# JuliaSmoothOptimizers/LinearOperators.jl

Hardware: AMD Instinct MI355X
Metric: mul! GB/s (frac HBM peak) at n=10^8 fp64; L-BFGS apply/s, 1/2/4/8 GPU (higher is better)
Workload: dtype f64; 1 GPU; opHouseholder(h) 5-arg mul!(res,H,v,1,0), n=100000000 fp64 per GPU (configs[1]); n_per_gpu=100000000, algorithmic_bytes_per_elt=40, devices_visible=1

## Files before the change

linearoperators.jl_amd/csrc/house_keep.h:

```cpp
#pragma once
#include "common.h"
#include "house_keep_plan.h"
#include "stream_kernels.h"

namespace mxlo {

constexpr int kHouseKeepKR = 14;
constexpr int kHouseKeepKL = 4;
constexpr int kHouseKeepUnroll = 4;
static_assert(kHouseKeepUnroll == kStreamUnroll, "the dot launch and the update launch count the same chunks");

constexpr int kHouseResidentNum = 14;
static_assert(kHouseResidentNum >= 0 && kHouseResidentNum <= 16);
#define MXLO_POLICY_SIDE(tag) asm volatile("; h loads: " tag ::: "memory")
struct HouseResident {
  int q = 0;
  int grid = 0;
};

template <typename T, typename CA, typename CB, bool BETA0, int KR, int KL>
__global__ void __launch_bounds__(kBlock)
householder_dots_keep_kernel(T *__restrict__ res, const T *__restrict__ h, const T *__restrict__ v, int64_t head,
                             int64_t n, CA alpha, CB beta, HouseKeepPlan pl, unsigned long long *__restrict__ slots,
                             unsigned long long ticks, unsigned *__restrict__ fault, int drop,
                             double *__restrict__ dot_out, int rq) {
  constexpr int VEC = Vec16<T>::N, U = kHouseKeepUnroll;
  using V = typename Vec16<T>::type;
  constexpr int64_t CHUNK = (int64_t)kBlock * U;
  extern __shared__ __attribute__((aligned(16))) unsigned char keep_lds[];
  V *lh = reinterpret_cast<V *>(keep_lds), *lx = lh + (int64_t)KL * CHUNK;
  const int tid = threadIdx.x, G = (int)gridDim.x, b = (int)blockIdx.x;
  GridExchange X;
  X.begin<kBlock>(slots, kFusedSlots);

  const V *hv = reinterpret_cast<const V *>(h + head), *xv = reinterpret_cast<const V *>(v + head);
  V *rv = reinterpret_cast<V *>(res + head);
  double acc = 0.0;
  auto load4 = [&](int64_t round, V (&a)[U], V (&x)[U]) {
    const int64_t base = (round * G + b) * CHUNK + tid;
    if (house_resident_diag((int)((round + b) & 15), rq)) {
      MXLO_POLICY_SIDE("resident");
#pragma unroll
      for (int u = 0; u < U; ++u) {
        x[u] = __builtin_nontemporal_load(xv + base + (int64_t)u * kBlock);
        a[u] = hv[base + (int64_t)u * kBlock];
      }
      MXLO_POLICY_SIDE("resident, issued");
    } else {
      MXLO_POLICY_SIDE("streamed");
#pragma unroll
      for (int u = 0; u < U; ++u) {
        x[u] = __builtin_nontemporal_load(xv + base + (int64_t)u * kBlock);
        a[u] = __builtin_nontemporal_load(hv + base + (int64_t)u * kBlock);
      }
      MXLO_POLICY_SIDE("streamed, issued");
    }
  };
  auto fma4 = [&](const V (&a)[U], const V (&x)[U]) {
#pragma unroll
    for (int u = 0; u < U; ++u)
#pragma unroll
      for (int k = 0; k < VEC; ++k) acc = fma((double)a[u][k], (double)x[u][k], acc);
  };
  for (int64_t r = 0; r < pl.first; ++r) {
    V a[U], x[U];
    load4(r, a, x);
    fma4(a, x);
  }
  if constexpr (KL > 0) {
#pragma unroll 1
    for (int q = 0; q < pl.kl; ++q) {
      V a[U], x[U];
      load4(pl.first + q, a, x);
      fma4(a, x);
#pragma unroll
      for (int u = 0; u < U; ++u) {
        lh[(q * U + u) * kBlock + tid] = a[u];
        lx[(q * U + u) * kBlock + tid] = x[u];
      }
    }
  }
  V kh[KR][U], kx[KR][U];
  const int64_t reg0 = pl.first + pl.kl;
#pragma unroll
  for (int q = 0; q < KR; ++q)
    if (q < pl.kr) load4(reg0 + q, kh[q], kx[q]);
#pragma unroll
  for (int q = 0; q < KR; ++q)
    if (q < pl.kr) fma4(kh[q], kx[q]);
  const int64_t rem = pl.rem_vec + (int64_t)b * CHUNK + tid;
#pragma unroll
  for (int u = 0; u < U; ++u) {
    const int64_t i = rem + (int64_t)u * kBlock;
    if (i < pl.nvec) {
      const V x = __builtin_nontemporal_load(xv + i), a = __builtin_nontemporal_load(hv + i);
#pragma unroll
      for (int k = 0; k < VEC; ++k) acc = fma((double)a[k], (double)x[k], acc);
    }
  }
  const int64_t tail0 = head + pl.nvec * VEC, cnt = head + (n - tail0);
  if (b == G - 1 && tid < cnt) {
    const int64_t i = tid < head ? tid : tail0 + (tid - head);
    acc = fma((double)h[i], (double)v[i], acc);
  }

  __shared__ double lds[kBlock / kWave];
  const double s = block_sum4(acc, lds);
  if (tid == 0) X.publish(b, s, b == drop);
  double p = 0.0;
  for (int i = tid; i < G; i += kBlock) p += X.wait(i, ticks, fault, kFaultHouseholder);
  __syncthreads();
  const double dot = block_sum4(p, lds);
  if (b == 0 && tid == 0) *dot_out = dot;
  X.finish();

  HouseholderOp<T, CA, CB, BETA0> op{alpha, beta, nullptr, T(0)};
  op.c = (T)2 * (T)dot;
  auto update4 = [&](int64_t round, const V (&a)[U], const V (&x)[U]) {
    const int64_t base = (round * G + b) * CHUNK + tid;
    V r[U];
    if constexpr (!BETA0) {
#pragma unroll
      for (int u = 0; u < U; ++u) r[u] = __builtin_nontemporal_load(rv + base + (int64_t)u * kBlock);
    }
#pragma unroll
    for (int u = 0; u < U; ++u) {
      V o;
#pragma unroll
      for (int k = 0; k < VEC; ++k) o[k] = op(a[u][k], x[u][k], BETA0 ? T(0) : r[u][k]);
      __builtin_nontemporal_store(o, rv + base + (int64_t)u * kBlock);
    }
  };
#pragma unroll
  for (int q = 0; q < KR; ++q)
    if (q < pl.kr) update4(reg0 + q, kh[q], kx[q]);
  if constexpr (KL > 0) {
#pragma unroll 1
    for (int q = 0; q < pl.kl; ++q) {
      V a[U], x[U];
#pragma unroll
      for (int u = 0; u < U; ++u) {
        a[u] = lh[(q * U + u) * kBlock + tid];
        x[u] = lx[(q * U + u) * kBlock + tid];
      }
      update4(pl.first + q, a, x);
    }
  }
#pragma unroll
  for (int u = 0; u < U; ++u) {
    const int64_t i = rem + (int64_t)u * kBlock;
    if (i < pl.nvec) {
      const V x = xv[i], a = hv[i];
      V r, o;
      if constexpr (!BETA0) r = rv[i];
#pragma unroll
      for (int k = 0; k < VEC; ++k) o[k] = op(a[k], x[k], BETA0 ? T(0) : r[k]);
      __builtin_nontemporal_store(o, rv + i);
    }
  }
  if (b == G - 1 && tid >= head && tid < cnt) {
    const int64_t i = tail0 + (tid - head);
    res[i] = op(h[i], v[i], BETA0 ? T(0) : res[i]);
  }
}

template <typename T>
static int32_t householder_dots_t(mxlo_ctx *ctx, T *res, const T *h, const T *v, int64_t *n_left, double alpha,
                                  double beta, int32_t flags, double *dot, HouseResident *rs) {
  constexpr int VEC = Vec16<T>::N, KR = kHouseKeepKR, KL = kHouseKeepKL;
  constexpr int64_t CHUNK = (int64_t)kBlock * kHouseKeepUnroll;
  constexpr size_t kLds = (size_t)2 * KL * CHUNK * 16;
  const int64_t n = *n_left;
  const T *cols[1] = {h};
  const int64_t head = common_head<T>({res, h, v});
  bool keep = ctx->tune.house_fused && !ctx->allreduce && ctx->fault_dev && n > ctx->tune.house_inline_n && head >= 0 &&
              n >= 4 * VEC && (int64_t)sizeof(T) * n * 2 >= ctx->tune.nt_min_bytes;
  HouseKeepPlan pl;
  int grid = 0;
  if (keep) {
    const int per_cu = ctx->tune.red_blocks_per_cu > 1 ? 1 : ctx->tune.red_blocks_per_cu;
    grid = grid_for(ctx, (n - head) / VEC, CHUNK, per_cu);
    pl = house_keep_plan(n, head, VEC, grid, CHUNK, KR, KL);
    keep = grid == ctx->num_cu && grid <= kFusedSlots && pl.ok;
  }
  if (!keep) return panel_dots<T>(ctx, cols, 1, v, n, dot);
  const int rq = house_resident_q((int64_t)sizeof(T) * n, ctx->tune.nt_min_bytes / 16 * kHouseResidentNum);
  bool launched = false;
  MXLO_TRY((dispatch_ab<T>(beta, flags, [&]<typename CA, typename CB, bool B0>() -> int32_t {
    constexpr auto kernel = householder_dots_keep_kernel<T, CA, CB, B0, KR, KL>;
    static std::atomic<int> lds_cap[64];
    const int d = ctx->device & 63;
    int st = kLds > 48 * 1024 ? lds_cap[d].load(std::memory_order_relaxed) : 1;
    if (st == 0) {
      st = hipFuncSetAttribute((const void *)kernel, hipFuncAttributeMaxDynamicSharedMemorySize, (int)kLds) == hipSuccess ? 1 : 2;
      if (st == 2) (void)hipGetLastError();
      lds_cap[d].store(st, std::memory_order_relaxed);
    }
    if (st != 1 || !coresident<kernel>(ctx, grid, kLds)) return MXLO_OK;
    hipLaunchKernelGGL(kernel, dim3(grid), dim3(kBlock), kLds, ctx->stream, res, h, v, head, n, (CA)alpha, (CB)beta, pl,
                       ctx->xslots, fused_timeout_ticks(ctx), ctx->fault_dev, ctx->tune.fused_debug_drop, dot, rq);
    MXLO_LAUNCH_CHECK();
    launched = true;
    return MXLO_OK;
  })));
  if (!launched) return panel_dots<T>(ctx, cols, 1, v, n, dot);
  *n_left = pl.prefix;
  *rs = HouseResident{rq, grid};
  return MXLO_OK;
}

template <typename T, typename CA, typename CB, bool BETA0, bool REVERSE, bool NT>
__global__ void __launch_bounds__(kBlock)
householder_update_resident_kernel(T *__restrict__ res, const T *__restrict__ h, const T *__restrict__ v, int64_t head,
                                   int64_t nchunks, int64_t dots_grid, int rq, HouseholderOp<T, CA, CB, BETA0> op) {
  constexpr int VEC = Vec16<T>::N, U = kStreamUnroll;
  using V = typename Vec16<T>::type;
  constexpr int64_t CHUNK = (int64_t)kBlock * U;
  op.init();
  const int tid = threadIdx.x;
  V *rv = reinterpret_cast<V *>(res + head);
  const V *hv = reinterpret_cast<const V *>(h + head), *xv = reinterpret_cast<const V *>(v + head);
  for (int64_t ch = blockIdx.x; ch < nchunks; ch += gridDim.x) {
    const int64_t c = REVERSE ? (nchunks - 1 - ch) : ch;
    const int64_t base = c * CHUNK + tid;
    V a[U], x[U], r[U];
    if (house_resident_chunk(c, dots_grid, rq)) {
      MXLO_POLICY_SIDE("resident");
#pragma unroll
      for (int u = 0; u < U; ++u) {
        a[u] = hv[base + (int64_t)u * kBlock];
        x[u] = ldg<NT>(xv + base + (int64_t)u * kBlock);
        if constexpr (!BETA0) r[u] = ldg<NT>(rv + base + (int64_t)u * kBlock);
      }
      MXLO_POLICY_SIDE("resident, issued");
    } else {
      MXLO_POLICY_SIDE("streamed");
#pragma unroll
      for (int u = 0; u < U; ++u) {
        a[u] = ldg<NT>(hv + base + (int64_t)u * kBlock);
        x[u] = ldg<NT>(xv + base + (int64_t)u * kBlock);
        if constexpr (!BETA0) r[u] = ldg<NT>(rv + base + (int64_t)u * kBlock);
      }
      MXLO_POLICY_SIDE("streamed, issued");
    }
#pragma unroll
    for (int u = 0; u < U; ++u) {
      V o;
#pragma unroll
      for (int k = 0; k < VEC; ++k) o[k] = op(a[u][k], x[u][k], BETA0 ? T(0) : r[u][k]);
      stg<NT>(rv + base + (int64_t)u * kBlock, o);
    }
  }
  if (blockIdx.x == gridDim.x - 1 && tid < head) res[tid] = op(h[tid], v[tid], BETA0 ? T(0) : res[tid]);
}

template <typename T>
static int32_t householder_apply_resident_t(mxlo_ctx *ctx, T *res, const T *h, const T *v, int64_t n, double alpha,
                                            double beta, int32_t flags, const double *dot, HouseResident rs) {
  constexpr int VEC = Vec16<T>::N;
  constexpr int64_t CHUNK = (int64_t)kBlock * kStreamUnroll;
  const int64_t head = common_head<T>({res, h, v}), nchunks = (n - head) / VEC / CHUNK;
  MXLO_REQUIRE(head >= 0 && rs.grid > 0 && head + nchunks * CHUNK * VEC == n, MXLO_ESTATE,
               "householder: the prefix of the kept form is not the scalar head and whole chunks");
  const bool rev = ctx->tune.house_reverse != 0;
  int64_t g = nchunks;
  if (ctx->tune.blocks_per_cu > 0 && g > (int64_t)ctx->num_cu * ctx->tune.blocks_per_cu) g = (int64_t)ctx->num_cu * ctx->tune.blocks_per_cu;
  const int grid = (int)(g > 0x7fffffffLL ? 0x7fffffffLL : (g < 1 ? 1 : g));
  return dispatch_ab<T>(beta, flags, [&]<typename CA, typename CB, bool B0>() -> int32_t {
    HouseholderOp<T, CA, CB, B0> op{(CA)alpha, (CB)beta, dot, T(0)};
    const bool nt = (int64_t)sizeof(T) * n * (B0 ? 3 : 4) >= ctx->tune.nt_min_bytes;
    auto go = [&]<bool REV, bool NT>() {
      hipLaunchKernelGGL((householder_update_resident_kernel<T, CA, CB, B0, REV, NT>), dim3(grid), dim3(kBlock), 0,
                         ctx->stream, res, h, v, head, nchunks, (int64_t)rs.grid, rs.q, op);
    };
    if (rev) nt ? go.template operator()<true, true>() : go.template operator()<true, false>();
    else nt ? go.template operator()<false, true>() : go.template operator()<false, false>();
    MXLO_LAUNCH_CHECK();
    return MXLO_OK;
  });
}

}
```

linearoperators.jl_amd/csrc/house_keep_plan.h:

```cpp
#pragma once
#include <cstdint>

namespace mxlo {

struct HouseKeepPlan {
  bool ok = false;
  int64_t rounds = 0;
  int64_t first = 0;
  int kl = 0, kr = 0;
  int64_t prefix = 0;
  int64_t rem_vec = 0;
  int64_t nvec = 0;
};

inline HouseKeepPlan house_keep_plan(int64_t n, int64_t head, int vec, int64_t grid, int64_t chunk, int KR, int KL) {
  HouseKeepPlan p;
  if (n < head || vec < 1 || grid < 1 || chunk < 1 || KR < 0 || KL < 0) return p;
  p.nvec = (n - head) / vec;
  p.rounds = p.nvec / chunk / grid;
  if (p.rounds < 2) return p;
  const int64_t kept = p.rounds - 1 < (int64_t)KR + KL ? p.rounds - 1 : (int64_t)KR + KL;
  p.kr = (int)(kept < KR ? kept : KR);
  p.kl = (int)(kept - p.kr);
  p.first = p.rounds - kept;
  p.prefix = head + p.first * grid * chunk * vec;
  p.rem_vec = p.rounds * grid * chunk;
  p.ok = kept >= 1;
  return p;
}


constexpr int house_resident_q(int64_t h_bytes, int64_t cache_bytes) {
  if (cache_bytes <= 0 || h_bytes < 0) return 0;
  if (h_bytes <= cache_bytes) return 16;
  return (int)(cache_bytes / ((h_bytes + 15) / 16));
}

constexpr bool house_resident_diag(int t, int q) { return (t * q) % 16 >= 16 - q; }
constexpr bool house_resident_chunk(int64_t c, int64_t grid, int q) {
  return house_resident_diag((int)(((c / grid) + (c % grid)) % 16), q);
}

}
```

linearoperators.jl_amd/csrc/leaves.hip:

```cpp
#include "common.h"
#include "stream_kernels.h"
#include "house_keep.h"
using namespace mxlo;

#define CHECK_COMMON(name)                                                                       \
  MXLO_REQUIRE(ctx != nullptr, MXLO_EINVAL, name ": ctx is NULL");                               \
  MXLO_REQUIRE(dtype == MXLO_F64 || dtype == MXLO_F32, MXLO_EINVAL, name ": bad dtype %d", dtype)

static inline double eff_beta(int32_t dtype, int32_t flags, double beta) {
  return beta_is_f64(dtype == MXLO_F64 ? 8 : 4, flags) ? beta : (double)(float)beta;
}
static inline double eff_alpha(int32_t dtype, int32_t flags, double alpha) {
  return alpha_is_f64(dtype == MXLO_F64 ? 8 : 4, flags) ? alpha : (double)(float)alpha;
}

template <typename T>
static int32_t fill(mxlo_ctx *ctx, T *p, int64_t n, T c) {
  if (n <= 0) return MXLO_OK;
  if (c == T(0)) {
    MXLO_HIP(hipMemsetAsync(p, 0, sizeof(T) * (size_t)n, ctx->stream));
    return MXLO_OK;
  }
  return launch_map<T, 0, false, false>(ctx, p, (const T *)nullptr, (const T *)nullptr, n,
                                        FillOp<T>{c});
// ... 25 lines not shown
               "mxlo_diag_mul: NULL operand");
  const int64_t es = dtype == MXLO_F64 ? 8 : 4;
  MXLO_TRY(stage_alias(ctx, res, nrow * es, &v, n_min * es, true, "mxlo_diag_mul"));
  alpha = eff_alpha(dtype, flags, alpha);
  beta = eff_beta(dtype, flags, beta);
  if (dtype == MXLO_F64)
    return diag_mul_t<double>(ctx, (double *)res, (const double *)d, (const double *)v, n_min, nrow,
                              alpha, beta, flags);
  return diag_mul_t<float>(ctx, (float *)res, (const float *)d, (const float *)v, n_min, nrow,
                           alpha, beta, flags);
}

template <typename T>
static int32_t eye_mul_t(mxlo_ctx *ctx, T *res, const T *v, int64_t n_min, int64_t nrow,
                         double alpha, double beta, int32_t flags) {
  int32_t st = dispatch_ab<T>(beta, flags, [&]<typename CA, typename CB, bool B0>() -> int32_t {
    AxpbyOp<T, CA, CB, B0> op{(CA)alpha, (CB)beta};
    return launch_map<T, 1, !B0, false>(ctx, res, v, (const T *)nullptr, n_min, op);
  });
  MXLO_TRY(st);
  const int64_t ntail = nrow - n_min;
  if (ntail <= 0) return MXLO_OK;
  if (beta == 0) return fill<T>(ctx, res + n_min, ntail, T(0));
  const bool f64s = beta_is_f64(sizeof(T), flags);
  if (flags & MXLO_TAIL_BETA) return fill<T>(ctx, res + n_min, ntail, (T)beta);
  if (f64s)
    return launch_map<T, 0, true, false>(ctx, res + n_min, (const T *)nullptr, (const T *)nullptr,
                                         ntail, ScaleOp<T, double>{beta});
  return launch_map<T, 0, true, false>(ctx, res + n_min, (const T *)nullptr, (const T *)nullptr,
                                       ntail, ScaleOp<T, float>{(float)beta});
}

MXLO_API int32_t mxlo_eye_mul(mxlo_ctx *ctx, int32_t dtype, void *res, const void *v,
                              int64_t n_min, int64_t nrow, double alpha, double beta,
                              int32_t flags) {
  CHECK_COMMON("mxlo_eye_mul");
  MXLO_DEVICE_GUARD(ctx);
  MXLO_REQUIRE(n_min >= 0 && nrow >= n_min, MXLO_ESHAPE, "mxlo_eye_mul: n_min=%lld nrow=%lld",
               (long long)n_min, (long long)nrow);
  MXLO_REQUIRE(nrow == 0 || (res && (n_min == 0 || v)), MXLO_EINVAL, "mxlo_eye_mul: NULL operand");
  const int64_t es = dtype == MXLO_F64 ? 8 : 4;
  MXLO_TRY(stage_alias(ctx, res, nrow * es, &v, n_min * es, true, "mxlo_eye_mul"));
  alpha = eff_alpha(dtype, flags, alpha);
  beta = eff_beta(dtype, flags, beta);
  if (dtype == MXLO_F64)
    return eye_mul_t<double>(ctx, (double *)res, (const double *)v, n_min, nrow, alpha, beta, flags);
  return eye_mul_t<float>(ctx, (float *)res, (const float *)v, n_min, nrow, alpha, beta, flags);
}

template <typename T>
static int32_t scale_t(mxlo_ctx *ctx, T *res, int64_t n, double s, bool f64s) {
  if (f64s)
    return launch_map<T, 0, true, false>(ctx, res, (const T *)nullptr, (const T *)nullptr, n,
                                         ScaleOp<T, double>{s});
  return launch_map<T, 0, true, false>(ctx, res, (const T *)nullptr, (const T *)nullptr, n,
                                       ScaleOp<T, float>{(float)s});
}

MXLO_API int32_t mxlo_zeros_mul(mxlo_ctx *ctx, int32_t dtype, void *res, int64_t nrow, double beta,
                                int32_t flags) {
  CHECK_COMMON("mxlo_zeros_mul");
  MXLO_DEVICE_GUARD(ctx);
  MXLO_REQUIRE(nrow >= 0 && (nrow == 0 || res), MXLO_EINVAL, "mxlo_zeros_mul: bad argument");
  beta = eff_beta(dtype, flags, beta);
  if (beta == 0) {
    if (dtype == MXLO_F64) return fill<double>(ctx, (double *)res, nrow, 0.0);
    return fill<float>(ctx, (float *)res, nrow, 0.f);
  }
  if (dtype == MXLO_F64) return scale_t<double>(ctx, (double *)res, nrow, beta, true);
  return scale_t<float>(ctx, (float *)res, nrow, beta, beta_is_f64(4, flags));
}

MXLO_API int32_t mxlo_fill(mxlo_ctx *ctx, int32_t dtype, void *res, int64_t n, double value) {
  CHECK_COMMON("mxlo_fill");
  MXLO_DEVICE_GUARD(ctx);
  MXLO_REQUIRE(n >= 0 && (n == 0 || res), MXLO_EINVAL, "mxlo_fill: bad argument");
  if (dtype == MXLO_F64) return fill<double>(ctx, (double *)res, n, value);
  return fill<float>(ctx, (float *)res, n, (float)value);
}

MXLO_API int32_t mxlo_scale(mxlo_ctx *ctx, int32_t dtype, void *res, int64_t n, double alpha,
                            int32_t flags) {
  CHECK_COMMON("mxlo_scale");
  MXLO_DEVICE_GUARD(ctx);
  MXLO_REQUIRE(n >= 0 && (n == 0 || res), MXLO_EINVAL, "mxlo_scale: bad argument");
  alpha = eff_alpha(dtype, flags, alpha);
  if (dtype == MXLO_F64) return scale_t<double>(ctx, (double *)res, n, alpha, true);
  return scale_t<float>(ctx, (float *)res, n, alpha, alpha_is_f64(4, flags));
}

namespace {
template <typename T>
__global__ void __launch_bounds__(kBlock)
sum_kernel(const T *__restrict__ v, int64_t n, double *__restrict__ partials) {
  constexpr int VEC = Vec16<T>::N;
  using V = typename Vec16<T>::type;
  double acc = 0.0;
  const int64_t head = (((uintptr_t)v & 15u) == 0) ? 0 : n;
  const int64_t nvec = head == 0 ? n / VEC : 0;
  const V *vv = reinterpret_cast<const V *>(v);
  const int64_t stride = (int64_t)gridDim.x * kBlock;
  int64_t i = (int64_t)blockIdx.x * kBlock + threadIdx.x;
  for (; i + 3 * stride < nvec; i += 4 * stride) {
    const V a = __builtin_nontemporal_load(vv + i), b = __builtin_nontemporal_load(vv + i + stride),
            c = __builtin_nontemporal_load(vv + i + 2 * stride), d = __builtin_nontemporal_load(vv + i + 3 * stride);
#pragma unroll
    for (int e = 0; e < VEC; ++e) acc += ((double)a[e] + (double)b[e]) + ((double)c[e] + (double)d[e]);
  }
  for (; i < nvec; i += stride) {
    const V a = vv[i];
#pragma unroll
    for (int e = 0; e < VEC; ++e) acc += (double)a[e];
  }
  for (int64_t k = nvec * VEC + (int64_t)blockIdx.x * kBlock + threadIdx.x; k < n; k += stride) acc += (double)v[k];
#pragma unroll
  for (int off = 32; off > 0; off >>= 1) acc += __shfl_down(acc, off, 64);
  __shared__ double lds[kBlock / kWave];
  if ((threadIdx.x & 63) == 0) lds[threadIdx.x >> 6] = acc;
  __syncthreads();
  if (threadIdx.x == 0) partials[blockIdx.x] = (lds[0] + lds[1]) + (lds[2] + lds[3]);
}
}

namespace mxlo {
int32_t allreduce_hook(mxlo_ctx *ctx, double *dev, int64_t count);
}

template <typename T>
static int32_t ones_mul_t(mxlo_ctx *ctx, T *res, int64_t nrow, const T *v, int64_t ncol,
                          double alpha, double beta, int32_t flags) {
  double *sum = ctx->scalars;
  if (ncol > 0) {
    const int grid = grid_for(ctx, ncol, kBlock * 8, ctx->tune.red_blocks_per_cu);
    hipLaunchKernelGGL((sum_kernel<T>), dim3(grid), dim3(kBlock), 0, ctx->stream, v, ncol,
                       ctx->partials);
    MXLO_LAUNCH_CHECK();
    MXLO_TRY(finalize_and_reduce(ctx, 1, grid, sum));
  } else {
    MXLO_HIP(hipMemsetAsync(sum, 0, sizeof(double), ctx->stream));
  }
  MXLO_TRY(allreduce_hook(ctx, sum, 1));
  return dispatch_ab<T>(beta, flags, [&]<typename CA, typename CB, bool B0>() -> int32_t {
    OnesOp<T, CA, CB, B0> op{(CA)alpha, (CB)beta, sum, (CA)0};
    return launch_map<T, 0, !B0, false>(ctx, res, (const T *)nullptr, (const T *)nullptr, nrow, op);
  });
}

MXLO_API int32_t mxlo_ones_mul(mxlo_ctx *ctx, int32_t dtype, void *res, int64_t nrow,
                               const void *v, int64_t ncol, double alpha, double beta,
                               int32_t flags) {
  CHECK_COMMON("mxlo_ones_mul");
  MXLO_DEVICE_GUARD(ctx);
  MXLO_REQUIRE(nrow >= 0 && ncol >= 0, MXLO_ESHAPE, "mxlo_ones_mul: negative size");
  alpha = eff_alpha(dtype, flags, alpha);
  beta = eff_beta(dtype, flags, beta);
  if (dtype == MXLO_F64)
    return ones_mul_t<double>(ctx, (double *)res, nrow, (const double *)v, ncol, alpha, beta, flags);
  return ones_mul_t<float>(ctx, (float *)res, nrow, (const float *)v, ncol, alpha, beta, flags);
}

template <typename T>
static int32_t householder_apply_t(mxlo_ctx *ctx, T *res, const T *h, const T *v, int64_t n,
                                   double alpha, double beta, int32_t flags, const double *dot) {
  const bool rev = ctx->tune.house_reverse != 0;
  return dispatch_ab<T>(beta, flags, [&]<typename CA, typename CB, bool B0>() -> int32_t {
    HouseholderOp<T, CA, CB, B0> op{(CA)alpha, (CB)beta, dot, T(0)};
    if (rev) return launch_map<T, 2, !B0, true>(ctx, res, h, v, n, op);
    return launch_map<T, 2, !B0, false>(ctx, res, h, v, n, op);
  });
}

namespace {
template <typename T, typename CA, typename CB, bool BETA0, int VPT, bool ALIGNED>
__global__ void __launch_bounds__(kBlock)
householder_fused_kernel(T *__restrict__ res, const T *__restrict__ h, const T *__restrict__ v, int64_t n, CA alpha,
                         CB beta, unsigned long long *__restrict__ slots, unsigned long long ticks,
                         unsigned *__restrict__ fault, int drop) {
  constexpr int VEC = Vec16<T>::N;
  using V = typename Vec16<T>::type;
  const int tid = threadIdx.x, G = (int)gridDim.x, b = (int)blockIdx.x;
  GridExchange X;
  X.begin<kBlock>(slots, kFusedSlots);

  T hh[VPT][VEC], vv[VPT][VEC];
  double acc = 0.0;
  const int64_t base = (int64_t)b * kBlock * VPT * VEC;
#pragma unroll
  for (int q = 0; q < VPT; ++q) {
    const int64_t i = base + ((int64_t)q * kBlock + tid) * VEC;
    if (ALIGNED && i + VEC <= n) {
      const V a = *reinterpret_cast<const V *>(h + i), c = *reinterpret_cast<const V *>(v + i);
#pragma unroll
      for (int k = 0; k < VEC; ++k) { hh[q][k] = a[k]; vv[q][k] = c[k]; }
    } else {
#pragma unroll
      for (int k = 0; k < VEC; ++k) {
        hh[q][k] = i + k < n ? h[i + k] : T(0);
        vv[q][k] = i + k < n ? v[i + k] : T(0);
      }
    }
  }
#pragma unroll
  for (int q = 0; q < VPT; ++q)
#pragma unroll
    for (int k = 0; k < VEC; ++k) acc = fma((double)hh[q][k], (double)vv[q][k], acc);

  __shared__ double lds[kBlock / kWave];
  const double s = block_sum4(acc, lds);
  if (tid == 0) X.publish(b, s, b == drop);
  double p = 0.0;
  if (tid < G) p = X.wait(tid, ticks, fault, kFaultHouseholder);
  if (tid + kBlock < G) p += X.wait(tid + kBlock, ticks, fault, kFaultHouseholder);
  __syncthreads();
  const double dot = block_sum4(p, lds);
  X.finish();

  HouseholderOp<T, CA, CB, BETA0> op{alpha, beta, nullptr, T(0)};
  op.c = (T)2 * (T)dot;
#pragma unroll
  for (int q = 0; q < VPT; ++q) {
    const int64_t i = base + ((int64_t)q * kBlock + tid) * VEC;
    if (ALIGNED && i + VEC <= n) {
      V r;
      if constexpr (!BETA0) r = *reinterpret_cast<const V *>(res + i);
      V o;
#pragma unroll
      for (int k = 0; k < VEC; ++k) o[k] = op(hh[q][k], vv[q][k], BETA0 ? T(0) : r[k]);
      *reinterpret_cast<V *>(res + i) = o;
    } else {
#pragma unroll
      for (int k = 0; k < VEC; ++k)
        if (i + k < n) res[i + k] = op(hh[q][k], vv[q][k], BETA0 ? T(0) : res[i + k]);
    }
  }
}
}

template <typename T>
static inline int64_t fused_grid(int64_t n, int vpt) {
  const int64_t per = (int64_t)kBlock * vpt * Vec16<T>::N;
  return (n + per - 1) / per;
}

template <typename T>
static int32_t householder_fused_t(mxlo_ctx *ctx, T *res, const T *h, const T *v, int64_t n, double alpha, double beta,
                                   int32_t flags, int vpt, bool *launched) {
  const bool aligned = ((((uintptr_t)res) | ((uintptr_t)h) | ((uintptr_t)v)) & 15u) == 0;
  const int grid = (int)fused_grid<T>(n, vpt);
  return dispatch_ab<T>(beta, flags, [&]<typename CA, typename CB, bool B0>() -> int32_t {
    bool fits = true;
    auto go = [&]<int VPT, bool AL>() {
      if (!(fits = coresident<householder_fused_kernel<T, CA, CB, B0, VPT, AL>>(ctx, grid))) return;
      hipLaunchKernelGGL((householder_fused_kernel<T, CA, CB, B0, VPT, AL>), dim3(grid), dim3(kBlock), 0, ctx->stream,
                         res, h, v, n, (CA)alpha, (CB)beta, ctx->xslots, fused_timeout_ticks(ctx), ctx->fault_dev,
                         ctx->tune.fused_debug_drop);
    };
    if (aligned) {
      if (vpt == 2) go.template operator()<2, true>();
      else if (vpt == 4) go.template operator()<4, true>();
      else if (vpt == 8) go.template operator()<8, true>();
      else go.template operator()<16, true>();
    } else {
      if (vpt == 2) go.template operator()<2, false>();
      else if (vpt == 4) go.template operator()<4, false>();
      else if (vpt == 8) go.template operator()<8, false>();
      else go.template operator()<16, false>();
    }
    *launched = fits;
    if (!fits) return MXLO_OK;
    MXLO_LAUNCH_CHECK();
    return MXLO_OK;
  });
}

template <typename T>
static int32_t householder_t(mxlo_ctx *ctx, T *res, const T *h, const T *v, int64_t n,
                             double alpha, double beta, int32_t flags) {
  if (ctx->tune.house_fused && !ctx->allreduce && n > 0 && ctx->fault_dev) {
    MXLO_TRY(fused_fault_check(ctx));
  }
  if (ctx->tune.house_fused && !ctx->allreduce && n > 0 && ctx->fault_dev) {
    const int64_t cap = std::min<int64_t>((int64_t)ctx->num_cu * (ctx->tune.house_fused_per_cu >= 2 ? 2 : 1), kFusedSlots);
    const int64_t cap1 = std::min<int64_t>(ctx->num_cu, kFusedSlots);
    const int vpt = fused_grid<T>(n, 2) <= 16 ? 2 : (fused_grid<T>(n, 4) <= 32 ? 4 : (fused_grid<T>(n, 8) <= cap1 ? 8 : 16));
    if (fused_grid<T>(n, vpt) <= cap) {
      bool launched = false;
      const int32_t st = householder_fused_t<T>(ctx, res, h, v, n, alpha, beta, flags, vpt, &launched);
      if (st != MXLO_OK || launched) return st;
    }
  }
  const T *cols[1] = {h};
  if (!ctx->allreduce && n >= 1 && n <= ctx->tune.house_inline_n) {
    int nb = 0;
    MXLO_TRY(panel_dots_partials<T>(ctx, cols, 1, v, n, &nb));
    const bool rev = ctx->tune.house_reverse != 0;
    return dispatch_ab<T>(beta, flags, [&]<typename CA, typename CB, bool B0>() -> int32_t {
      HouseholderPartialsOp<T, CA, CB, B0> op{(CA)alpha, (CB)beta, ctx->partials, nb, T(0)};
      if (rev) return launch_map<T, 2, !B0, true>(ctx, res, h, v, n, op);
      return launch_map<T, 2, !B0, false>(ctx, res, h, v, n, op);
    });
  }
  double *dot = ctx->scalars;
  HouseResident rs; MXLO_TRY(householder_dots_t<T>(ctx, res, h, v, &n, alpha, beta, flags, dot, &rs));
  return rs.q > 0 ? householder_apply_resident_t<T>(ctx, res, h, v, n, alpha, beta, flags, dot, rs) : householder_apply_t<T>(ctx, res, h, v, n, alpha, beta, flags, dot);
}

MXLO_API int32_t mxlo_dot(mxlo_ctx *ctx, int32_t dtype, const void *a, const void *b, int64_t n,
                          double *out_dev) {
  CHECK_COMMON("mxlo_dot");
  MXLO_DEVICE_GUARD(ctx);
  MXLO_REQUIRE(n >= 0 && out_dev && (n == 0 || (a && b)), MXLO_EINVAL, "mxlo_dot: bad argument");
  if (dtype == MXLO_F64) {
    const double *cols[1] = {(const double *)a};
    return panel_dots<double>(ctx, cols, 1, (const double *)b, n, out_dev);
  }
  const float *cols[1] = {(const float *)a};
  return panel_dots<float>(ctx, cols, 1, (const float *)b, n, out_dev);
}

MXLO_API int32_t mxlo_householder_apply(mxlo_ctx *ctx, int32_t dtype, void *res, const void *h,
                                        const void *v, int64_t n, double alpha, double beta,
                                        int32_t flags, const double *dot_dev) {
  CHECK_COMMON("mxlo_householder_apply");
  MXLO_DEVICE_GUARD(ctx);
  MXLO_REQUIRE(n >= 0 && dot_dev && (n == 0 || (res && h && v)), MXLO_EINVAL,
               "mxlo_householder_apply: bad argument");
  MXLO_TRY(stage_alias(ctx, res, n * (dtype == MXLO_F64 ? 8 : 4), &v, n * (dtype == MXLO_F64 ? 8 : 4), true,
                       "mxlo_householder_apply"));
  alpha = eff_alpha(dtype, flags, alpha);
  beta = eff_beta(dtype, flags, beta);
  if (dtype == MXLO_F64)
    return householder_apply_t<double>(ctx, (double *)res, (const double *)h, (const double *)v, n,
                                       alpha, beta, flags, dot_dev);
  return householder_apply_t<float>(ctx, (float *)res, (const float *)h, (const float *)v, n, alpha,
                                    beta, flags, dot_dev);
}

MXLO_API int32_t mxlo_householder_mul(mxlo_ctx *ctx, int32_t dtype, void *res, const void *h,
                                      const void *v, int64_t n, double alpha, double beta,
                                      int32_t flags) {
  CHECK_COMMON("mxlo_householder_mul");
  MXLO_DEVICE_GUARD(ctx);
  MXLO_REQUIRE(n >= 0 && (n == 0 || (res && h && v)), MXLO_EINVAL,
               "mxlo_householder_mul: bad argument");
  MXLO_TRY(stage_alias(ctx, res, n * (dtype == MXLO_F64 ? 8 : 4), &v, n * (dtype == MXLO_F64 ? 8 : 4), true,
                       "mxlo_householder_mul"));
  alpha = eff_alpha(dtype, flags, alpha);
  beta = eff_beta(dtype, flags, beta);
  if (dtype == MXLO_F64)
    return householder_t<double>(ctx, (double *)res, (const double *)h, (const double *)v, n, alpha,
                                 beta, flags);
  return householder_t<float>(ctx, (float *)res, (const float *)h, (const float *)v, n, alpha, beta,
                              flags);
}

namespace {
template <typename T>
struct CopyBitsOp {
  __device__ void init() {}
  __device__ T operator()(T x, T, T) const { return x; }
};

typedef unsigned int u32;
typedef unsigned long long u64;
typedef u64 u64x2 __attribute__((ext_vector_type(2)));

template <typename E, bool VECOUT>
__global__ void __launch_bounds__(kBlock)
gather_idx_kernel(E *__restrict__ res, const E *__restrict__ v, const int64_t *__restrict__ idx,
                  int64_t nidx) {
  constexpr int KPT = sizeof(E) >= 16 ? 1 : 16 / (int)sizeof(E);
  constexpr int U = 4;
  typedef long long i64x2 __attribute__((ext_vector_type(2)));
  const int64_t ngroups = (nidx + KPT - 1) / KPT;
  const bool idx_al = (((uintptr_t)idx) & 15u) == 0;
  for (int64_t base = ((int64_t)blockIdx.x * U) * kBlock + threadIdx.x; base < ngroups;
       base += (int64_t)gridDim.x * U * kBlock) {
    int64_t j[U][KPT];
#pragma unroll
    for (int u = 0; u < U; ++u) {
      const int64_t k0 = (base + (int64_t)u * kBlock) * KPT;
      if (KPT >= 2 && idx_al && k0 + KPT <= nidx) {
#pragma unroll
        for (int q = 0; q < KPT; q += 2) {
          const i64x2 t = __builtin_nontemporal_load(reinterpret_cast<const i64x2 *>(idx + k0 + q));
          j[u][q] = t[0] - 1;
          j[u][q + (KPT >= 2 ? 1 : 0)] = t[1] - 1;
        }
      } else {
#pragma unroll
        for (int q = 0; q < KPT; ++q) j[u][q] = k0 + q < nidx ? idx[k0 + q] - 1 : 0;
      }
    }
    E e[U][KPT];
#pragma unroll
    for (int u = 0; u < U; ++u)
#pragma unroll
      for (int q = 0; q < KPT; ++q) e[u][q] = v[j[u][q]];
#pragma unroll
    for (int u = 0; u < U; ++u) {
      const int64_t k0 = (base + (int64_t)u * kBlock) * KPT;
      if (VECOUT && k0 + KPT <= nidx) {
        struct alignas(16) Pack { E x[KPT]; };
        Pack p;
#pragma unroll
        for (int q = 0; q < KPT; ++q) p.x[q] = e[u][q];
        typedef unsigned int u32x4 __attribute__((ext_vector_type(4)));
        __builtin_nontemporal_store(*reinterpret_cast<u32x4 *>(&p), reinterpret_cast<u32x4 *>(res + k0));
      } else {
#pragma unroll
        for (int q = 0; q < KPT; ++q)
          if (k0 + q < nidx) res[k0 + q] = e[u][q];
      }
    }
  }
}

template <typename E>
__global__ void __launch_bounds__(kBlock)
gather_range_kernel(E *__restrict__ res, const E *__restrict__ v, int64_t start0, int64_t step,
                    int64_t len, int32_t res_aligned) {
  constexpr int VEC = sizeof(E) >= 16 ? 1 : 16 / (int)sizeof(E);
  const int64_t ngroups = (len + VEC - 1) / VEC;
  for (int64_t g = (int64_t)blockIdx.x * kBlock + threadIdx.x; g < ngroups; g += (int64_t)gridDim.x * kBlock) {
    const int64_t k0 = g * VEC;
    const E *src = v + start0 + k0 * step;
    if (k0 + VEC <= len) {
      struct alignas(16) Pack { E x[VEC]; };
      Pack pk;
#pragma unroll
      for (int q = 0; q < VEC; ++q) pk.x[q] = src[(int64_t)q * step];
      if (res_aligned) {
        typedef unsigned int u32x4 __attribute__((ext_vector_type(4)));
        __builtin_nontemporal_store(*reinterpret_cast<u32x4 *>(&pk), reinterpret_cast<u32x4 *>(res + k0));
      } else {
#pragma unroll
        for (int q = 0; q < VEC; ++q) res[k0 + q] = pk.x[q];
      }
    } else {
      for (int q = 0; k0 + q < len; ++q) res[k0 + q] = src[(int64_t)q * step];
    }
  }
}

template <typename E>
__global__ void __launch_bounds__(kBlock)
scatter_idx_kernel(E *__restrict__ res, const E *__restrict__ u, const int64_t *__restrict__ idx,
                   const int64_t *__restrict__ pos, int64_t nidx) {
  for (int64_t k = (int64_t)blockIdx.x * kBlock + threadIdx.x; k < nidx;
       k += (int64_t)gridDim.x * kBlock) {
    const int64_t src = pos ? pos[k] : k;
    res[idx[k] - 1] = u[src];
  }
}

template <typename E>
__global__ void __launch_bounds__(kBlock)
extend_range_kernel(E *__restrict__ res, int64_t nres, const E *__restrict__ u, int64_t start0,
                    int64_t step, int64_t len, int64_t sq, int64_t sr, int32_t res_aligned) {
  constexpr int VEC = sizeof(E) >= 16 ? 1 : 16 / (int)sizeof(E);
  const int64_t stop0 = start0 + (len - 1) * step;
  const int64_t lo = step > 0 ? start0 : stop0, hi = step > 0 ? stop0 : start0;
  const int64_t astep = step > 0 ? step : -step;
  const int64_t ngroups = (nres + VEC - 1) / VEC;
  int64_t g = (int64_t)blockIdx.x * kBlock + threadIdx.x;
  if (g >= ngroups) return;
  int64_t off = g * VEC - lo;
  int64_t q = off >= 0 ? off / astep : -((-off + astep - 1) / astep);
  int64_t r = off - q * astep;
  for (; g < ngroups; g += (int64_t)gridDim.x * kBlock) {
    const int64_t i0 = g * VEC;
    struct alignas(16) Pack { E x[VEC]; };
    Pack pk;
    int64_t qq = q, rr = r;
#pragma unroll
    for (int j = 0; j < VEC; ++j) {
      E val;
      memset(&val, 0, sizeof(E));
      const int64_t i = i0 + j;
      if (rr == 0 && len > 0 && i >= lo && i <= hi) val = u[step > 0 ? qq : (len - 1) - qq];
      pk.x[j] = val;
      if (++rr == astep) { rr = 0; ++qq; }
    }
    if (res_aligned && i0 + VEC <= nres) {
      typedef unsigned int u32x4 __attribute__((ext_vector_type(4)));
      __builtin_nontemporal_store(*reinterpret_cast<u32x4 *>(&pk), reinterpret_cast<u32x4 *>(res + i0));
    } else {
#pragma unroll
      for (int j = 0; j < VEC; ++j)
        if (i0 + j < nres) res[i0 + j] = pk.x[j];
    }
    q += sq;
    r += sr;
    if (r >= astep) { r -= astep; ++q; }
  }
}

__device__ __forceinline__ int64_t wave_lower_bound(const int64_t *__restrict__ idx, int64_t lo, int64_t hi,
                                                    int64_t target, int lane) {
  while (true) {
    const int64_t n = hi - lo;
    if (n <= 0) return lo;
    if (n <= 64) {
      const int64_t p = lo + lane;
      const bool lt = p < hi && idx[p] < target;
      return lo + __popcll(__ballot(lt));
    }
    const int64_t p = lo + ((int64_t)(lane + 1) * n) / 65;
    const bool lt = idx[p] < target;
    const int c = __popcll(__ballot(lt));
    const int64_t nlo = c == 0 ? lo : lo + ((int64_t)c * n) / 65 + 1;
    const int64_t nhi = c == 64 ? hi : lo + ((int64_t)(c + 1) * n) / 65;
    lo = nlo;
    hi = nhi;
  }
}

template <typename E, int TILE_BYTES>
__global__ void __launch_bounds__(kBlock)
extend_sorted_kernel(E *__restrict__ res, int64_t nres, const E *__restrict__ u, const int64_t *__restrict__ idx,
                     const int64_t *__restrict__ pos, int64_t nidx, int64_t ntiles, int32_t tiles_per_block,
                     int32_t res_aligned) {
  constexpr int TILE = TILE_BYTES / (int)sizeof(E);
  typedef unsigned int u32x4 __attribute__((ext_vector_type(4)));
  __shared__ u32x4 smem[TILE_BYTES / 16];
  __shared__ int64_t bounds[2];
  E *tile = reinterpret_cast<E *>(smem);
  const int tid = threadIdx.x;
  const int64_t tb = (int64_t)blockIdx.x * tiles_per_block;
  const int64_t te = tb + tiles_per_block < ntiles ? tb + tiles_per_block : ntiles;
  const u32x4 z = {0u, 0u, 0u, 0u};
  int64_t s = 0;
  for (int64_t t = tb; t < te; ++t) {
    const int64_t t0 = t * TILE, t1 = t0 + TILE < nres ? t0 + TILE : nres;
    if (tid < 64) {
      if (t == tb) s = wave_lower_bound(idx, 0, nidx, t0 + 1, tid);
      const int64_t cap = s + TILE < nidx ? s + TILE : nidx;
      const int64_t e = wave_lower_bound(idx, s, cap, t1 + 1, tid);
      if (tid == 0) { bounds[0] = s; bounds[1] = e; }
    }
#pragma unroll
    for (int w = tid; w < TILE_BYTES / 16; w += kBlock) smem[w] = z;
    __syncthreads();
    s = bounds[0];
    const int64_t e = bounds[1];
    for (int64_t k = s + tid; k < e; k += kBlock) {
      const int64_t j = idx[k] - 1 - t0;
      const E val = u[pos ? pos[k] : k];
      if (j >= 0 && j < t1 - t0) tile[j] = val;
    }
    s = e;
    __syncthreads();
    const int64_t nbytes = (t1 - t0) * (int64_t)sizeof(E);
    if (res_aligned) {
      u32x4 *dst = reinterpret_cast<u32x4 *>(res + t0);
      const int nv = (int)(nbytes / 16);
      for (int w = tid; w < nv; w += kBlock) __builtin_nontemporal_store(smem[w], dst + w);
      for (int64_t j = (int64_t)nv * (16 / (int)sizeof(E)) + tid; j < t1 - t0; j += kBlock) res[t0 + j] = tile[j];
    } else {
      for (int64_t j = tid; j < t1 - t0; j += kBlock) res[t0 + j] = tile[j];
    }
    __syncthreads();
  }
}

template <typename F>
int32_t by_elem_size(int32_t es, F &&f) {
  switch (es) {
    case 4: return f.template operator()<u32>();
    case 8: return f.template operator()<u64>();
    case 16: return f.template operator()<u64x2>();
    default: set_error("element size %d not in {4,8,16}", es); return MXLO_EINVAL;
  }
}
}

MXLO_API int32_t mxlo_gather(mxlo_ctx *ctx, int32_t elem_size, void *res, const void *v,
                             int64_t nv, const int64_t *idx, int64_t nidx) {
  MXLO_REQUIRE(ctx, MXLO_EINVAL, "mxlo_gather: ctx is NULL");
  MXLO_DEVICE_GUARD(ctx);
  MXLO_REQUIRE(nidx >= 0 && nv >= 0, MXLO_ESHAPE, "mxlo_gather: negative size");
  if (nidx == 0) return MXLO_OK;
  MXLO_REQUIRE(res && v && idx, MXLO_EINVAL, "mxlo_gather: NULL operand");
  MXLO_REQUIRE(elem_size == 4 || elem_size == 8 || elem_size == 16, MXLO_EINVAL, "element size %d not in {4,8,16}", elem_size);
  MXLO_TRY(stage_alias(ctx, res, nidx * elem_size, &v, nv * elem_size, false, "mxlo_gather"));
  return by_elem_size(elem_size, [&]<typename E>() -> int32_t {
    constexpr int KPT = sizeof(E) >= 16 ? 1 : 16 / (int)sizeof(E);
    const int grid = grid_for(ctx, (nidx + KPT - 1) / KPT, kBlock * 4, ctx->tune.blocks_per_cu);
    if ((((uintptr_t)res) & 15u) == 0)
      hipLaunchKernelGGL((gather_idx_kernel<E, true>), dim3(grid), dim3(kBlock), 0, ctx->stream, (E *)res,
                         (const E *)v, idx, nidx);
    else
      hipLaunchKernelGGL((gather_idx_kernel<E, false>), dim3(grid), dim3(kBlock), 0, ctx->stream, (E *)res,
                         (const E *)v, idx, nidx);
    MXLO_LAUNCH_CHECK();
    return MXLO_OK;
  });
}

MXLO_API int32_t mxlo_gather_range(mxlo_ctx *ctx, int32_t elem_size, void *res, const void *v,
                                   int64_t nv, int64_t start, int64_t step, int64_t len) {
  MXLO_REQUIRE(ctx, MXLO_EINVAL, "mxlo_gather_range: ctx is NULL");
  MXLO_DEVICE_GUARD(ctx);
  MXLO_REQUIRE(len >= 0 && nv >= 0, MXLO_ESHAPE, "mxlo_gather_range: negative size");
  if (len == 0) return MXLO_OK;
  MXLO_REQUIRE(res && v, MXLO_EINVAL, "mxlo_gather_range: NULL operand");
  const int64_t last = start + (len - 1) * step;
// ... 411 lines not shown
```

Before: 7217 GB/s.

## Plan cache-resident h chunks at finer granularity with partial diagonal fill

```diff
diff --git a/linearoperators.jl_amd/csrc/house_keep.h b/linearoperators.jl_amd/csrc/house_keep.h
--- a/linearoperators.jl_amd/csrc/house_keep.h
+++ b/linearoperators.jl_amd/csrc/house_keep.h
@@ -10,20 +10,16 @@
 constexpr int kHouseKeepUnroll = 4;
 static_assert(kHouseKeepUnroll == kStreamUnroll, "the dot launch and the update launch count the same chunks");
 
-constexpr int kHouseResidentNum = 14;
-static_assert(kHouseResidentNum >= 0 && kHouseResidentNum <= 16);
+constexpr int kHouseResidentNum = 240;
+static_assert(kHouseResidentNum >= 0 && kHouseResidentNum <= 256);
 #define MXLO_POLICY_SIDE(tag) asm volatile("; h loads: " tag ::: "memory")
-struct HouseResident {
-  int q = 0;
-  int grid = 0;
-};
 
 template <typename T, typename CA, typename CB, bool BETA0, int KR, int KL>
 __global__ void __launch_bounds__(kBlock)
 householder_dots_keep_kernel(T *__restrict__ res, const T *__restrict__ h, const T *__restrict__ v, int64_t head,
                              int64_t n, CA alpha, CB beta, HouseKeepPlan pl, unsigned long long *__restrict__ slots,
                              unsigned long long ticks, unsigned *__restrict__ fault, int drop,
-                             double *__restrict__ dot_out, int rq) {
+                             double *__restrict__ dot_out, HouseResident rs) {
   constexpr int VEC = Vec16<T>::N, U = kHouseKeepUnroll;
   using V = typename Vec16<T>::type;
   constexpr int64_t CHUNK = (int64_t)kBlock * U;
@@ -36,9 +32,9 @@
   const V *hv = reinterpret_cast<const V *>(h + head), *xv = reinterpret_cast<const V *>(v + head);
   V *rv = reinterpret_cast<V *>(res + head);
   double acc = 0.0;
-  auto load4 = [&](int64_t round, V (&a)[U], V (&x)[U]) {
+  auto load4 = [&](int64_t round, V (&a)[U], V (&x)[U], bool prefix) {
     const int64_t base = (round * G + b) * CHUNK + tid;
-    if (house_resident_diag((int)((round + b) & 15), rq)) {
+    if (prefix && house_resident_at(round, b, rs)) {
       MXLO_POLICY_SIDE("resident");
 #pragma unroll
       for (int u = 0; u < U; ++u) {
@@ -64,14 +60,14 @@
   };
   for (int64_t r = 0; r < pl.first; ++r) {
     V a[U], x[U];
-    load4(r, a, x);
+    load4(r, a, x, true);
     fma4(a, x);
   }
   if constexpr (KL > 0) {
 #pragma unroll 1
     for (int q = 0; q < pl.kl; ++q) {
       V a[U], x[U];
-      load4(pl.first + q, a, x);
+      load4(pl.first + q, a, x, false);
       fma4(a, x);
 #pragma unroll
       for (int u = 0; u < U; ++u) {
@@ -84,7 +80,7 @@
   const int64_t reg0 = pl.first + pl.kl;
 #pragma unroll
   for (int q = 0; q < KR; ++q)
-    if (q < pl.kr) load4(reg0 + q, kh[q], kx[q]);
+    if (q < pl.kr) load4(reg0 + q, kh[q], kx[q], false);
 #pragma unroll
   for (int q = 0; q < KR; ++q)
     if (q < pl.kr) fma4(kh[q], kx[q]);
@@ -184,7 +180,7 @@
     keep = grid == ctx->num_cu && grid <= kFusedSlots && pl.ok;
   }
   if (!keep) return panel_dots<T>(ctx, cols, 1, v, n, dot);
-  const int rq = house_resident_q((int64_t)sizeof(T) * n, ctx->tune.nt_min_bytes / 16 * kHouseResidentNum);
+  const HouseResident slice = house_resident_plan(pl.first, grid, CHUNK * 16, ctx->tune.nt_min_bytes / 256 * kHouseResidentNum);
   bool launched = false;
   MXLO_TRY((dispatch_ab<T>(beta, flags, [&]<typename CA, typename CB, bool B0>() -> int32_t {
     constexpr auto kernel = householder_dots_keep_kernel<T, CA, CB, B0, KR, KL>;
@@ -198,21 +194,21 @@
     }
     if (st != 1 || !coresident<kernel>(ctx, grid, kLds)) return MXLO_OK;
     hipLaunchKernelGGL(kernel, dim3(grid), dim3(kBlock), kLds, ctx->stream, res, h, v, head, n, (CA)alpha, (CB)beta, pl,
-                       ctx->xslots, fused_timeout_ticks(ctx), ctx->fault_dev, ctx->tune.fused_debug_drop, dot, rq);
+                       ctx->xslots, fused_timeout_ticks(ctx), ctx->fault_dev, ctx->tune.fused_debug_drop, dot, slice);
     MXLO_LAUNCH_CHECK();
     launched = true;
     return MXLO_OK;
   })));
   if (!launched) return panel_dots<T>(ctx, cols, 1, v, n, dot);
   *n_left = pl.prefix;
-  *rs = HouseResident{rq, grid};
+  *rs = slice;
   return MXLO_OK;
 }
 
 template <typename T, typename CA, typename CB, bool BETA0, bool REVERSE, bool NT>
 __global__ void __launch_bounds__(kBlock)
 householder_update_resident_kernel(T *__restrict__ res, const T *__restrict__ h, const T *__restrict__ v, int64_t head,
-                                   int64_t nchunks, int64_t dots_grid, int rq, HouseholderOp<T, CA, CB, BETA0> op) {
+                                   int64_t nchunks, HouseResident rs, HouseholderOp<T, CA, CB, BETA0> op) {
   constexpr int VEC = Vec16<T>::N, U = kStreamUnroll;
   using V = typename Vec16<T>::type;
   constexpr int64_t CHUNK = (int64_t)kBlock * U;
@@ -224,7 +220,7 @@
     const int64_t c = REVERSE ? (nchunks - 1 - ch) : ch;
     const int64_t base = c * CHUNK + tid;
     V a[U], x[U], r[U];
-    if (house_resident_chunk(c, dots_grid, rq)) {
+    if (house_resident(c, rs)) {
       MXLO_POLICY_SIDE("resident");
 #pragma unroll
       for (int u = 0; u < U; ++u) {
@@ -260,7 +256,8 @@
   constexpr int VEC = Vec16<T>::N;
   constexpr int64_t CHUNK = (int64_t)kBlock * kStreamUnroll;
   const int64_t head = common_head<T>({res, h, v}), nchunks = (n - head) / VEC / CHUNK;
-  MXLO_REQUIRE(head >= 0 && rs.grid > 0 && head + nchunks * CHUNK * VEC == n, MXLO_ESTATE,
+  MXLO_REQUIRE(head >= 0 && rs.grid > 0 && nchunks == rs.rounds * rs.grid && head + nchunks * CHUNK * VEC == n,
+               MXLO_ESTATE,
                "householder: the prefix of the kept form is not the scalar head and whole chunks");
   const bool rev = ctx->tune.house_reverse != 0;
   int64_t g = nchunks;
@@ -271,7 +268,7 @@
     const bool nt = (int64_t)sizeof(T) * n * (B0 ? 3 : 4) >= ctx->tune.nt_min_bytes;
     auto go = [&]<bool REV, bool NT>() {
       hipLaunchKernelGGL((householder_update_resident_kernel<T, CA, CB, B0, REV, NT>), dim3(grid), dim3(kBlock), 0,
-                         ctx->stream, res, h, v, head, nchunks, (int64_t)rs.grid, rs.q, op);
+                         ctx->stream, res, h, v, head, nchunks, rs, op);
     };
     if (rev) nt ? go.template operator()<true, true>() : go.template operator()<true, false>();
     else nt ? go.template operator()<false, true>() : go.template operator()<false, false>();
diff --git a/linearoperators.jl_amd/csrc/house_keep_plan.h b/linearoperators.jl_amd/csrc/house_keep_plan.h
--- a/linearoperators.jl_amd/csrc/house_keep_plan.h
+++ b/linearoperators.jl_amd/csrc/house_keep_plan.h
@@ -41,4 +41,90 @@
   return house_resident_diag((int)(((c / grid) + (c % grid)) % 16), q);
 }
 
+struct HouseResident {
+  uint32_t mask = 0;
+  int32_t q = 0;
+  int32_t t = 0;
+  uint64_t step = 0;
+  int64_t grid = 0;
+  int64_t rounds = 0;
+  int64_t chunks = 0;
+  constexpr bool any() const { return chunks > 0; }
+};
+
+constexpr int64_t house_resident_before(int64_t grid, int t, int rho) {
+  const int64_t off = 16 - ((t - rho + 17) & 15);
+  return ((grid + off) / 16 - off / 16) * rho + ((grid + off) % 16 < rho ? (grid + off) % 16 : rho) -
+         (off % 16 < rho ? off % 16 : rho);
 }
+
+constexpr bool house_resident_at(int64_t round, int64_t wg, const HouseResident &rs) {
+  if (round >= rs.rounds) return false;
+  const int t = (int)((round + wg) & 15);
+  if ((rs.mask >> t) & 1u) return true;
+  if (t != rs.t || rs.step == 0) return false;
+  const uint32_t i = (uint32_t)((round >> 4) * rs.grid + house_resident_before(rs.grid, t, (int)(round & 15)) + (wg >> 4));
+  return (((uint64_t)(uint32_t)(i * (uint32_t)rs.step) + rs.step) >> 32) != 0;
+}
+constexpr bool house_resident(int64_t c, const HouseResident &rs) { return house_resident_at(c / rs.grid, c % rs.grid, rs); }
+
+inline HouseResident house_resident_plan(int64_t rounds, int64_t grid, int64_t chunk_bytes, int64_t budget_bytes) {
+  HouseResident rs;
+  if (rounds < 1 || grid < 1 || chunk_bytes < 1) return rs;
+  rs.grid = grid;
+  rs.rounds = rounds;
+  const int64_t all = rounds * grid, want = budget_bytes / chunk_bytes;
+  if (want <= 0) return rs;
+  if (want >= all) {
+    rs.mask = 0xffffu, rs.q = 16, rs.chunks = all;
+    return rs;
+  }
+  int64_t len[16];
+  for (int t = 0; t < 16; ++t)
+    len[t] = (rounds / 16) * grid + house_resident_before(grid, t, (int)(rounds % 16));
+  auto count = [&](uint32_t m) {
+    int64_t s = 0;
+    for (int t = 0; t < 16; ++t) s += (m >> t) & 1u ? len[t] : 0;
+    return s;
+  };
+  auto diagonals = [](int q) {
+    uint32_t m = 0;
+    for (int t = 0; t < 16; ++t) m |= house_resident_diag(t, q) ? 1u << t : 0u;
+    return m;
+  };
+  rs.q = house_resident_q(all * chunk_bytes, want * chunk_bytes);
+  while (rs.q > 0 && count(diagonals(rs.q)) > want) --rs.q;
+  rs.mask = diagonals(rs.q);
+  rs.chunks = count(rs.mask);
+  uint32_t extra = 0;
+  for (;;) {
+    int best = -1, gap = -1;
+    for (int t = 0; t < 16; ++t) {
+      if (((rs.mask >> t) & 1u) || len[t] == 0) continue;
+      int lo = 1, hi = 1;
+      while (lo < 16 && !((rs.mask >> ((t - lo) & 15)) & 1u)) ++lo;
+      while (hi < 16 && !((rs.mask >> ((t + hi) & 15)) & 1u)) ++hi;
+      int ex = 8;
+      for (int e = 1; e < 8; ++e)
+        if ((((extra >> ((t - e) & 15)) | (extra >> ((t + e) & 15))) & 1u) && e < ex) ex = e;
+      const int d = 256 * (lo < hi ? lo : hi) + 16 * ex + lo + hi;
+      if (d > gap) gap = d, best = t;
+    }
+    if (best < 0) break;
+    extra |= 1u << best;
+    const int64_t room = want - rs.chunks;
+    if (room >= len[best]) {
+      rs.mask |= 1u << best, rs.chunks += len[best];
+      continue;
+    }
+    if (room > 0 && len[best] < ((int64_t)1 << 32)) {
+      rs.t = best;
+      rs.step = (((uint64_t)room << 32) + (uint64_t)len[best] - 1) / (uint64_t)len[best];
+      rs.chunks += room;
+    }
+    break;
+  }
+  return rs;
+}
+
+}
diff --git a/linearoperators.jl_amd/csrc/leaves.hip b/linearoperators.jl_amd/csrc/leaves.hip
--- a/linearoperators.jl_amd/csrc/leaves.hip
+++ b/linearoperators.jl_amd/csrc/leaves.hip
@@ -351,7 +351,7 @@
   }
   double *dot = ctx->scalars;
   HouseResident rs; MXLO_TRY(householder_dots_t<T>(ctx, res, h, v, &n, alpha, beta, flags, dot, &rs));
-  return rs.q > 0 ? householder_apply_resident_t<T>(ctx, res, h, v, n, alpha, beta, flags, dot, rs) : householder_apply_t<T>(ctx, res, h, v, n, alpha, beta, flags, dot);
+  return rs.any() ? householder_apply_resident_t<T>(ctx, res, h, v, n, alpha, beta, flags, dot, rs) : householder_apply_t<T>(ctx, res, h, v, n, alpha, beta, flags, dot);
 }
 
 MXLO_API int32_t mxlo_dot(mxlo_ctx *ctx, int32_t dtype, const void *a, const void *b, int64_t n,
```

Result: no change. 7278 GB/s (median of 6 runs) (+0.8%).
